# jmhb0/view_neti

Hardware: AMD Instinct MI355X
Metric: TI train steps/sec (SD-1.5 512^2 bs=4 per GPU) (higher is better)
Workload: dtype f16; 1 GPU; learnable_mode 0, sd15 shapes, 512x512 fp16, bs=4/GPU, grad_accum 1, full train step (VAE+16xCLIP+UNet fwd/bwd+AdamW); global_batch=4, parallelism=dp1, rccl_ranks=1, hipgraph=True

## Files before the change

### view_neti_amd/csrc/gemm8.hip

```cpp
#include <type_traits>

#include "common.h"
#include "gemm_args.h"

namespace {

constexpr int BM = 256, NT = 512;
constexpr int HALF_BYTES = 128 * 128;
constexpr int GN_IMG = 5;

#define VN_WAIT_VM(n) asm volatile("s_waitcnt vmcnt(" #n ")" ::: "memory")
#define VN_WAIT_LGKM0() asm volatile("s_waitcnt lgkmcnt(0)" ::: "memory")

template <int BN, int EPI, bool CONV, bool HALO = false>
__global__ __launch_bounds__(NT) void gemm8_kernel(GemmArgs g) {
  static_assert(BN == 256 || BN == 128, "tile width");
  static_assert(!HALO || (BN == 128 && CONV), "the halo-patch loop exists for the 256x128 convolution tile");
  constexpr int PATCH_STRIDE = 41 * 1024;
  constexpr bool H42 = HALO && BN == 128;
  constexpr int NJB = BN / 128;
  constexpr int HB_BYTES = (BN / 2) * 128;
  constexpr int HB_DMA = BN / 128;
  constexpr int NBUF = BN == 256 ? 2 : 3;
  constexpr int BUF_BYTES = 2 * HALF_BYTES + 2 * HB_BYTES;
// ... 633 lines not shown
        }
      }
      if (EPI == 2 && e_gate) {
        const long long go = (long long)m * g.ld_gate + (e_geglu == 2 ? 2 * n : n);
        gv[u] = as_half8(vn_buf_load16_once(rsG, ok ? (uint32_t)(go * 2) : VN_OOB));
        gv2[u] = as_half8(vn_buf_load16_once(rsG, (ok && e_geglu == 2) ? (uint32_t)(go * 2 + 16) : VN_OOB));
      }
    }
#pragma unroll
    for (int u = 0; u < U; ++u) {
      const int r = r_first + RPP * (it0 + u);
      const int m = rowmem(r);
      const bool valid = m < g.M && n < g.N;
      if (gn && !gn_one) {
        int img = gn_img;
        if (valid) {
          img = (int)((float)m * rcp_gnhw);
          const int rem = m - img * g.gn_hw;
          img += rem >= g.gn_hw ? 1 : (rem < 0 ? -1 : 0);
        }
        if (__any(img != gn_img)) {
          gn_flush();
          gn_img = img;
        }
      }
      if (!valid) continue;
      half8 v = cv[u];
      if (full_chunk) {
        if (EPI >= 1 && e_rowadd) {
          v = vn_add8(v, av[u]);
        }
        if (Rb) {
          v = vn_add8(v, rv[u]);
        }
        if (e_geglu == 2) {
#pragma unroll
          for (int c2 = 0; c2 < 2; ++c2) {
            const half8 pre = c2 == 0 ? gv[u] : gv2[u];
            half8 o;
#pragma unroll
            for (int e = 0; e < 4; ++e) {
              const float d = (float)v[4 * c2 + e], hh = (float)pre[e], gg = (float)pre[4 + e];
              float cdf, xpdf;
              vn_gelu_parts(gg, cdf, xpdf);
              o[e] = (half_t)(d * gg * cdf);
              o[4 + e] = (half_t)(d * hh * (cdf + xpdf));
            }
            vn_st16_wt(rsC, (uint32_t)(((long long)m * g.ldc + 2 * n + 8 * c2) * 2), o);
          }
          continue;
        }
        if (e_gate) {
#pragma unroll
          for (int e = 0; e < 8; ++e) v[e] = (half_t)((float)v[e] * act_grad((float)gv[u][e], g.gate_act));
        }
        if (e_geglu == 1 || (e_C2 && e_geglu == 0)) vn_st16_wt_saved(rsC, (uint32_t)(((long long)m * g.ldc + n) * 2), v);
        else vn_st16_wt(rsC, (uint32_t)(((long long)m * g.ldc + n) * 2), v);
        if (e_geglu == 1) {
          half4 o2;
#pragma unroll
          for (int e = 0; e < 4; ++e) o2[e] = (half_t)((float)v[e] * vn_gelu_erf((float)v[4 + e]));
          *reinterpret_cast<half4*>(e_C2 + (long long)m * g.ldc2 + (n >> 1)) = o2;
        }
        if (gn) {
          {
            const half2v one2 = {(half_t)1.f, (half_t)1.f};
#pragma unroll
            for (int e = 0; e < 8; e += 2) {
              const half2v p2 = {v[e], v[e + 1]};
              if (e < gn_split) {
                s_lo = VN_FDOT2(p2, one2, s_lo);
                q_lo = VN_FDOT2(p2, p2, q_lo);
              } else {
                s_hi = VN_FDOT2(p2, one2, s_hi);
                q_hi = VN_FDOT2(p2, p2, q_hi);
              }
            }
          }
        }
        if (e_C2 && e_geglu == 0) {
          half8 o2;
#pragma unroll
          for (int e = 0; e < 8; ++e) o2[e] = (half_t)apply_act((float)v[e], g.act2);
          vn_st16_wt(rsC2, (uint32_t)(((long long)m * g.ldc2 + n) * 2), o2);
        }
      } else {
        const half_t* radd = e_rowadd ? e_rowadd + (long long)(m / g.rows_per_group) * g.ld_rowadd + n : nullptr;
        for (int e = 0; e < 8 && n + e < g.N; ++e) {
          float x = (float)v[e];
          if (radd) x = (float)(half_t)(x + (float)radd[e]);
          if (Rb) x = (float)(half_t)(x + (float)Rb[(long long)m * g.ldr + n + e]);
          if (e_gate) x = (float)(half_t)(x * act_grad((float)e_gate[(long long)m * g.ld_gate + n + e], g.gate_act));
          Cb[(long long)m * g.ldc + n + e] = (half_t)x;
          if (e_C2) e_C2[(long long)m * g.ldc2 + n + e] = (half_t)apply_act((float)(half_t)x, g.act2);
          if (gn) {
            const float xs = (float)(half_t)x;
            if (e < gn_split) {
              s_lo += xs;
              q_lo += xs * xs;
            } else {
              s_hi += xs;
              q_hi += xs * xs;
            }
          }
        }
      }
    }
  }
  if (gn_one) {
    float v4[4] = {s_lo, q_lo, s_hi, q_hi};
#pragma unroll
    for (int k = 0; k < 4; ++k) {
      v4[k] += __shfl_xor(v4[k], 32);
      v4[k] += __shfl_xor(v4[k], 16);
    }
    static_assert(CPR == 16 || !HALO, "the halo tile is 128 columns wide");
    float* tab = reinterpret_cast<float*>(smem + LDS_BYTES);
    if (lane < 16) *reinterpret_cast<f32x4*>(tab + (wave * 16 + lane) * 4) = f32x4{v4[0], v4[1], v4[2], v4[3]};
    __syncthreads();
    if (tid < 32) {
      const int col = tid >> 1, half = tid & 1;
      float sv = 0.f, qv = 0.f;
#pragma unroll
      for (int w8 = 0; w8 < 8; ++w8) {
        sv += tab[(w8 * 16 + col) * 4 + 2 * half];
        qv += tab[(w8 * 16 + col) * 4 + 2 * half + 1];
      }
      const int nc = n0 + col * 8;
      const int glo = nc / g.gn_cpg;
      const int split = (glo + 1) * g.gn_cpg - nc;
      if (nc < g.N && (half == 0 || split < 8)) {
        const int slot = tile_m % g.gn_slots;
        vn_u64* dst = reinterpret_cast<vn_u64*>(e_gn_sums) + (((long long)hb * g.gn_slots + slot) * g.gn_G + glo + half) * 4;
        vn_fx_add2(dst, sv, qv);
      }
    }
  } else if (gn) {
    gn_flush();
    __syncthreads();
    const int slot = tile_m % g.gn_slots;
    for (int i = tid; i < GN_IMG * GN_NG; i += NT) {
      const vn_u64* src = gacc + 4 * i;
      if ((src[0] | src[1] | src[2] | src[3]) == 0) continue;
      const int img = gn_img0 + i / GN_NG, grp = gn_g0t + i % GN_NG;
      vn_u64* dst = reinterpret_cast<vn_u64*>(e_gn_sums) + (((long long)img * g.gn_slots + slot) * g.gn_G + grp) * 4;
#pragma unroll
      for (int w = 0; w < 4; ++w) atomicAdd(dst + w, src[w]);
    }
  }
}

inline int epilogue_level8(const GemmArgs& g) {
  if (g.gate_src || g.C2 || g.geglu || g.act) return 2;
  return (g.gn_sums || g.rowadd) ? 1 : 0;
}

}

int vneti_launch_gemm8(void* gemm_args, int bn, int halo, hipStream_t st) {
  GemmArgs& g = *reinterpret_cast<GemmArgs*>(gemm_args);
  if (g.out_f32 || (g.conv_mode && (g.ups || (g.conv_mode == 2 && g.stride == 2))) ||
      (g.M >= (1 << 24) && (g.conv_mode || g.rowadd || g.gn_sums)))
    return VNETI_EUNSUP;
  if (halo && (bn != 128 || g.conv_mode < 1 || g.conv_mode > 2 || g.stride != 1 || g.pad_t != 1 || g.pad_l != 1 || g.Hi != g.Ho ||
               g.Wi != g.Wo || (g.Ho & 15) || (g.Wo & 15) || (g.Ci & 63) || g.K != 9 * g.Ci || !g.korder ||
               g.batch != 1 || g.M != (g.M / (g.Ho * g.Wo)) * g.Ho * g.Wo))
    return VNETI_EUNSUP;
  if (halo && g.ksplit > 1) {
    const int nchunk = g.Ci / 64, cps = cdiv(nchunk, g.ksplit);
    g.kt_per_split = 9 * cps;
    g.ksplit = cdiv(nchunk, cps);
  }
  g.tiles_m = cdiv(g.M, BM);
  g.tiles_n = cdiv(g.N, bn);
  const dim3 grid(g.tiles_m * g.tiles_n, g.batch, g.ksplit), block(NT);
  const int epi = epilogue_level8(g);
#define VN_GO(E, C)                                                                        \
  do {                                                                                     \
    if (bn == 256) hipLaunchKernelGGL((gemm8_kernel<256, E, C>), grid, block, 0, st, g);   \
    else hipLaunchKernelGGL((gemm8_kernel<128, E, C>), grid, block, 0, st, g);             \
  } while (0)
#define VN_GO_HALO(E) hipLaunchKernelGGL((gemm8_kernel<128, E, true, true>), grid, block, 0, st, g)
  if (halo) {
    if (epi == 2) VN_GO_HALO(2); else if (epi == 1) VN_GO_HALO(1); else VN_GO_HALO(0);
  } else if (g.conv_mode) {
    if (epi == 2) VN_GO(2, true); else if (epi == 1) VN_GO(1, true); else VN_GO(0, true);
  } else {
    if (epi == 2) VN_GO(2, false); else if (epi == 1) VN_GO(1, false); else VN_GO(0, false);
  }
#undef VN_GO
#undef VN_GO_HALO
  return vneti_check_launch("gemm8_kernel");
}
```

### view_neti_amd/csrc/gemm_conv.hip

```cpp
#include "common.h"
#include "gemm_args.h"
#include "../../include/vneti.h"

namespace {

template <int BM, int BN, int WM, int WN, bool F32OUT, bool DMA, int NSTG = 2, int EPI = 2, bool CONV = true>
__global__ __launch_bounds__((BM / WM) * (BN / WN) * 64) void gemm_kernel(
    const half_t* pA, const half_t* pB, uint32_t p_a_bytes, uint32_t p_b_bytes, int p_lda, int p_ldb, int pM, int pN, int pK,
    int p_tiles_m, int p_tiles_n, int p_split_conv , const GemmArgs gfull) {
  GemmArgs g = gfull;
  g.A = pA;
  g.B = pB;
  g.a_bytes = p_a_bytes;
  g.b_bytes = p_b_bytes;
  g.lda = p_lda;
  g.ldb = p_ldb;
  g.M = pM;
  g.N = pN;
  g.K = pK;
  g.tiles_m = p_tiles_m;
  g.tiles_n = p_tiles_n;
  g.kt_per_split = p_split_conv & 0xffff;
  g.ksplit = (p_split_conv >> 16) & 0xff;
  g.conv_mode = p_split_conv >> 24;
// ... 466 lines not shown
              s_lo += x;
              q_lo += x * x;
            } else {
              s_hi += x;
              q_hi += x * x;
            }
          }
        }
        if (e_C2 && e_geglu == 0) {
          half8 o2;
#pragma unroll
          for (int e = 0; e < 8; ++e) o2[e] = (half_t)apply_act((float)v[e], g.act2);
          vn_st16_wt(rsC2, (uint32_t)(((long long)m * g.ldc2 + n) * 2), o2);
        }
      } else {
        for (int e = 0; e < 8 && n + e < g.N; ++e) {
          float x = (float)v[e];
          if (radd) x = (float)(half_t)(x + (float)radd[e]);
          if (Rb) x = (float)(half_t)(x + (float)Rb[(long long)m * g.ldr + n + e]);
          if (e_gate) x = (float)(half_t)(x * act_grad((float)e_gate[(long long)m * g.ld_gate + n + e], g.gate_act));
          Cb[(long long)m * g.ldc + n + e] = (half_t)x;
          if (e_C2) e_C2[(long long)m * g.ldc2 + n + e] = (half_t)apply_act((float)(half_t)x, g.act2);
          if (gn) {
            const float xs = (float)(half_t)x;
            if (e < gn_split) {
              s_lo += xs;
              q_lo += xs * xs;
            } else {
              s_hi += xs;
              q_hi += xs * xs;
            }
          }
        }
      }
    }
    if (gn) {
      gn_flush();
      __syncthreads();
      const int slot = tile_m % g.gn_slots;
      for (int i = tid; i < GN_IMG * GN_NG; i += NT) {
        const vn_u64* src = gacc + 4 * i;
        if ((src[0] | src[1] | src[2] | src[3]) == 0) continue;
        const int img = gn_img0 + i / GN_NG, grp = gn_g0t + i % GN_NG;
        vn_u64* dst = reinterpret_cast<vn_u64*>(e_gn_sums) + (((long long)img * g.gn_slots + slot) * g.gn_G + grp) * 4;
#pragma unroll
        for (int w = 0; w < 4; ++w) atomicAdd(dst + w, src[w]);
      }
    }
  }
}

__global__ __launch_bounds__(256) void splitk_reduce_kernel(
    float* p_ws, void* pC, const float* p_bias, const void* p_resid, const half_t* p_rowadd, int pM, int pN, int p_batch,
    int p_ksplit, int p_ldc, int p_ldr, const GemmArgs gfull) {
  GemmArgs g = gfull;
  g.ws = p_ws;
  g.C = pC;
  g.bias = p_bias;
  g.resid = p_resid;
  g.rowadd = p_rowadd;
  g.M = pM;
  g.N = pN;
  g.batch = p_batch;
  g.ksplit = p_ksplit;
  g.ldc = p_ldc;
  g.ldr = p_ldr;
  const unsigned n4 = (unsigned)(g.N + 3) / 4;
  const unsigned gid = blockIdx.x * 256u + threadIdx.x;
  const unsigned total = (unsigned)g.batch * (unsigned)g.M * n4;
  if (gid >= total) return;
  const unsigned row = gid / n4;
  const int c = (int)(gid - row * n4) * 4;
  const int bz = g.batch > 1 ? (int)(row / (unsigned)g.M) : 0;
  const int m = (int)(row - (unsigned)bz * (unsigned)g.M);
  const int ne = min(4, g.N - c);
  const long long zstride = (long long)g.batch * g.M * g.N;
  const float* p0 = g.ws + ((long long)bz * g.M + m) * g.N + c;
  if ((g.N & 3) == 0 && ((g.ldc | g.ldr | g.ld_rowadd | g.ld_gate | g.ldc2) & 3) == 0) {
    const long long co = (long long)bz * g.strideC + (long long)m * g.ldc + c;
    const long long ro = (long long)bz * g.strideC + (long long)m * g.ldr + c;
    f32x4 bv = {0.f, 0.f, 0.f, 0.f}, rf = {0.f, 0.f, 0.f, 0.f};
    half4 rh = {0, 0, 0, 0}, ra = {0, 0, 0, 0}, gt = {0, 0, 0, 0};
    if (g.bias) bv = *reinterpret_cast<const f32x4*>(g.bias + c);
    if (g.resid) {
      if (g.out_f32) rf = *reinterpret_cast<const f32x4*>(reinterpret_cast<const float*>(g.resid) + ro);
      else rh = *reinterpret_cast<const half4*>(reinterpret_cast<const half_t*>(g.resid) + ro);
    }
    if (g.rowadd) ra = *reinterpret_cast<const half4*>(g.rowadd + (long long)(m / g.rows_per_group) * g.ld_rowadd + c);
    if (g.gate_src) gt = *reinterpret_cast<const half4*>(g.gate_src + (long long)m * g.ld_gate + c);
    f32x4 v = {0.f, 0.f, 0.f, 0.f};
    int z = 0;
    for (; z + 4 <= g.ksplit; z += 4) {
      const f32x4 t0 = *reinterpret_cast<const f32x4*>(p0 + (z + 0) * zstride);
      const f32x4 t1 = *reinterpret_cast<const f32x4*>(p0 + (z + 1) * zstride);
      const f32x4 t2 = *reinterpret_cast<const f32x4*>(p0 + (z + 2) * zstride);
      const f32x4 t3 = *reinterpret_cast<const f32x4*>(p0 + (z + 3) * zstride);
      v += t0;
      v += t1;
      v += t2;
      v += t3;
    }
    for (; z < g.ksplit; ++z) v += *reinterpret_cast<const f32x4*>(p0 + z * zstride);
    float x[4];
#pragma unroll
    for (int e = 0; e < 4; ++e) {
      x[e] = v[e] * g.alpha;
      if (g.bias) x[e] += bv[e];
      x[e] = apply_act(x[e], g.act);
    }
    if (g.out_f32) {
      f32x4 o = {x[0], x[1], x[2], x[3]};
      if (g.resid) o += rf;
      vn_st16_wt(vn_make_rsrc(g.C, 0x7fffffffu), (uint32_t)(co * 4), o);
    } else {
      half4 o, o2;
#pragma unroll
      for (int e = 0; e < 4; ++e) {
        float y = (float)(half_t)x[e];
        if (g.rowadd) y = (float)(half_t)(y + (float)ra[e]);
        if (g.resid) y = (float)(half_t)(y + (float)rh[e]);
        if (g.gate_src) y = (float)(half_t)(y * act_grad((float)gt[e], g.gate_act));
        o[e] = (half_t)y;
        o2[e] = (half_t)apply_act((float)(half_t)y, g.act2);
      }
      *reinterpret_cast<half4*>(reinterpret_cast<half_t*>(g.C) + co) = o;
      if (g.C2) *reinterpret_cast<half4*>(g.C2 + (long long)m * g.ldc2 + c) = o2;
    }
    return;
  }
  float v[4] = {0.f, 0.f, 0.f, 0.f};
  for (int z = 0; z < g.ksplit; ++z) {
    const float* p = p0 + z * zstride;
    for (int e = 0; e < ne; ++e) v[e] += p[e];
  }
  for (int e = 0; e < ne; ++e) {
    float x = v[e] * g.alpha;
    if (g.bias) x += g.bias[c + e];
    x = apply_act(x, g.act);
    if (g.out_f32) {
      if (g.resid) x += reinterpret_cast<const float*>(g.resid)[(long long)bz * g.strideC + (long long)m * g.ldr + c + e];
      reinterpret_cast<float*>(g.C)[(long long)bz * g.strideC + (long long)m * g.ldc + c + e] = x;
    } else {
      x = (float)(half_t)x;
      if (g.rowadd) x = (float)(half_t)(x + (float)g.rowadd[(long long)(m / g.rows_per_group) * g.ld_rowadd + c + e]);
      if (g.resid)
        x = (float)(half_t)(x + (float)reinterpret_cast<const half_t*>(g.resid)[(long long)bz * g.strideC + (long long)m * g.ldr + c + e]);
      if (g.gate_src) x = (float)(half_t)(x * act_grad((float)g.gate_src[(long long)m * g.ld_gate + c + e], g.gate_act));
      reinterpret_cast<half_t*>(g.C)[(long long)bz * g.strideC + (long long)m * g.ldc + c + e] = (half_t)x;
      if (g.C2) g.C2[(long long)m * g.ldc2 + c + e] = (half_t)apply_act((float)(half_t)x, g.act2);
    }
  }
}

inline int epilogue_level(const GemmArgs& g) {
  if (g.gate_src || g.C2 || g.geglu || g.act) return 2;
  return (g.gn_sums || g.rowadd) ? 1 : 0;
}

template <int BM, int BN, int WM, int WN, bool F32OUT, bool DMA, int NSTG>
void launch_variant(const GemmArgs& g, dim3 grid, hipStream_t st) {
  const dim3 block((BM / WM) * (BN / WN) * 64);
#define VN_GO(E, C)                                                                                                        \
  hipLaunchKernelGGL((gemm_kernel<BM, BN, WM, WN, F32OUT, DMA, NSTG, E, C>), grid, block, 0, st, g.A, g.B, g.a_bytes, g.b_bytes, \
                     (int)g.lda, (int)g.ldb, g.M, g.N, g.K, g.tiles_m, g.tiles_n, g.kt_per_split | (g.ksplit << 16) | (g.conv_mode << 24), g)
  if constexpr (F32OUT) {
    if (g.conv_mode) { if (g.act) VN_GO(2, true); else VN_GO(0, true); }
    else { if (g.act) VN_GO(2, false); else VN_GO(0, false); }
  } else {
    const int epi = epilogue_level(g);
    if (g.conv_mode) { if (epi == 2) VN_GO(2, true); else if (epi == 1) VN_GO(1, true); else VN_GO(0, true); }
    else { if (epi == 2) VN_GO(2, false); else if (epi == 1) VN_GO(1, false); else VN_GO(0, false); }
  }
#undef VN_GO
}

inline void launch_reduce(const GemmArgs& g, hipStream_t st) {
  if (g.ksplit > 1) {
    long long total = (long long)g.batch * g.M * ((g.N + 3) / 4);
    hipLaunchKernelGGL(splitk_reduce_kernel, dim3((unsigned)cdivl(total, 256)), dim3(256), 0, st, g.ws, g.C, g.bias, g.resid,
                       g.rowadd, g.M, g.N, g.batch, g.ksplit, (int)g.ldc, (int)g.ldr, g);
  }
}

template <int BM, int BN, int WM, int WN, bool DMA>
int launch_cfg(GemmArgs& g, bool f32out, hipStream_t st) {
  g.tiles_m = cdiv(g.M, BM);
  g.tiles_n = cdiv(g.N, BN);
  dim3 grid(g.tiles_m * g.tiles_n, g.batch, g.ksplit);
  if (f32out) launch_variant<BM, BN, WM, WN, true, DMA, 2>(g, grid, st);
  else launch_variant<BM, BN, WM, WN, false, DMA, 2>(g, grid, st);
  launch_reduce(g, st);
  return vneti_check_launch("gemm_kernel");
}

template <int BM, int BN, int WM, int WN, int NSTG = 3>
int launch_cfg_ring(GemmArgs& g, bool f32out, hipStream_t st) {
  g.tiles_m = cdiv(g.M, BM);
  g.tiles_n = cdiv(g.N, BN);
  dim3 grid(g.tiles_m * g.tiles_n, g.batch, g.ksplit);
  if (f32out) launch_variant<BM, BN, WM, WN, true, true, NSTG>(g, grid, st);
  else launch_variant<BM, BN, WM, WN, false, true, NSTG>(g, grid, st);
  launch_reduce(g, st);
  return vneti_check_launch("gemm_kernel");
}

template <int BM, int BN, int WM, int WN, bool DMA>
int launch_cfg_f16(GemmArgs& g, hipStream_t st) {
  g.tiles_m = cdiv(g.M, BM);
  g.tiles_n = cdiv(g.N, BN);
  dim3 grid(g.tiles_m * g.tiles_n, g.batch, g.ksplit);
  launch_variant<BM, BN, WM, WN, false, DMA, 2>(g, grid, st);
  launch_reduce(g, st);
  return vneti_check_launch("gemm_kernel");
}

struct TileDims {
  int bm, bn;
};
constexpr int kMaxTile = 18;
constexpr TileDims kTiles[kMaxTile + 1] = {{0, 0},     {128, 128}, {128, 64},  {64, 64},  {256, 128}, {256, 256}, {256, 128}, {256, 128},
                                          {256, 128}, {128, 128}, {128, 128}, {128, 64},  {64, 64},   {128, 128}, {128, 64},  {64, 64},
                                          {256, 256}, {256, 128}, {256, 128}};

int select_tile(int M, int N, int batch) {
  long long t256 = (long long)cdiv(M, 256) * cdiv(N, 128) * batch;
  long long t128 = (long long)cdiv(M, 128) * cdiv(N, 128) * batch;
  long long t12864 = (long long)cdiv(M, 128) * cdiv(N, 64) * batch;
  if (N <= 64) return (M >= 2048) ? 2 : 3;
  (void)t256;
  if (t128 >= 384) return 1;
  if (t12864 >= 384) return 2;
  return 3;
}

int select_ksplit(int M, int N, int K, int batch, int tile, long long ws_floats) {
  if (ws_floats <= 0) return 1;
  const int nk = K / 64;
  long long tiles = (long long)cdiv(M, kTiles[tile].bm) * cdiv(N, kTiles[tile].bn) * batch;
  if (tiles >= 256 || nk < 16) return 1;
  int s = (int)(512 / tiles);
  if (s > nk / 8) s = nk / 8;
  if (s > 16) s = 16;
  while (s > 1 && (long long)s * batch * M * N > ws_floats) --s;
  return s < 2 ? 1 : s;
}

}

extern "C" int vneti_gemm_select_tile(int M, int N, int batch) { return select_tile(M, N, batch > 0 ? batch : 1); }

extern "C" int vneti_gemm_select_split(int M, int N, int K, int batch, int tile_hint, long long workspace_bytes) {
  if (batch <= 0) batch = 1;
  int cfg = tile_hint >= 100 ? tile_hint - 100 : tile_hint;
  if (cfg == 0) cfg = select_tile(M, N, batch);
  if (cfg < 1 || cfg > kMaxTile || K % 64 != 0) return -1;
  int ks = select_ksplit(M, N, K, batch, cfg, workspace_bytes / 4);
  const int nk = K / 64;
  if (ks > nk) ks = nk;
  if (ks < 1) ks = 1;
  return cdiv(nk, cdiv(nk, ks));
}

extern "C" int vneti_gemm_f16(const vneti_gemm_desc* d, void* stream) {
  VN_REQUIRE(d != nullptr, "gemm: null descriptor");
  VN_REQUIRE(d->A && d->B && d->C, "gemm: null operand pointer");
  VN_REQUIRE(d->M > 0 && d->N > 0 && d->K > 0, "gemm: bad shape M=%d N=%d K=%d", d->M, d->N, d->K);
  VN_REQUIRE(d->K % 64 == 0, "gemm: K=%d must be a multiple of 64", d->K);
  VN_REQUIRE(d->ldb % 8 == 0, "gemm: ldb=%lld must be a multiple of 8", d->ldb);
  int batch = d->batch > 0 ? d->batch : 1;
  GemmArgs g;
  memset(&g, 0, sizeof(g));
  g.A = (const half_t*)d->A;
  g.B = (const half_t*)d->B;
  g.C = d->C;
  g.bias = d->bias;
  g.rowadd = (const half_t*)d->rowadd;
  g.resid = d->resid;
  g.gate_src = (const half_t*)d->gate_src;
  g.ld_gate = d->ld_gate;
  g.gate_act = d->gate_act;
  g.C2 = (half_t*)d->C2;
  g.ldc2 = d->ldc2;
  g.act2 = d->act2;
  g.gn_sums = (float*)d->gn_sums;
  g.gn_hw = d->gn_hw;
  g.gn_cpg = d->gn_cpg;
  g.gn_G = d->gn_groups;
  g.gn_slots = d->gn_slots;
  g.geglu = d->geglu;
  g.lda = d->lda;
  g.ldb = d->ldb;
  g.ldc = d->ldc;
  g.ld_rowadd = d->ld_rowadd;
  g.ldr = d->ldr;
  g.strideA = d->strideA;
  g.strideB = d->strideB;
  g.strideC = d->strideC;
  g.M = d->M;
  g.N = d->N;
  g.K = d->K;
  g.batch = batch;
  g.rows_per_group = d->rows_per_group > 0 ? d->rows_per_group : 1;
  g.alpha = d->alpha;
  g.act = d->act;
  g.out_f32 = d->out_f32 ? 1 : 0;
  g.conv_mode = d->conv_mode;
  long long a_bytes;
  if (d->conv_mode == 0) {
    VN_REQUIRE(d->lda % 8 == 0, "gemm: lda=%lld must be a multiple of 8", d->lda);
    a_bytes = ((long long)(d->M - 1) * d->lda + d->K) * 2;
  } else {
    VN_REQUIRE(d->conv_mode == 1 || d->conv_mode == 2, "gemm: bad conv_mode %d", d->conv_mode);
    VN_REQUIRE(d->Ci > 0 && d->Ci % 64 == 0, "conv: Ci=%d must be a multiple of 64", d->Ci);
    VN_REQUIRE(d->K == 9 * d->Ci, "conv: K=%d must equal 9*Ci=%d", d->K, 9 * d->Ci);
    VN_REQUIRE(d->stride == 1 || d->stride == 2, "conv: stride %d unsupported", d->stride);
    VN_REQUIRE(d->Ho > 0 && d->Wo > 0 && d->M % (d->Ho * d->Wo) == 0, "conv: M=%d not a multiple of Ho*Wo", d->M);
    VN_REQUIRE(d->ldx % 8 == 0, "conv: ldx must be a multiple of 8");
    VN_REQUIRE(!(d->ups && d->conv_mode != 1), "conv: fused upsample only in forward gather mode");
    VN_REQUIRE(!(d->ups && d->stride != 1), "conv: fused upsample needs stride 1");
    g.Hi = d->Hi;
    g.Wi = d->Wi;
    g.Ci = d->Ci;
    g.Ho = d->Ho;
    g.Wo = d->Wo;
    g.stride = d->stride;
    g.pad_t = d->pad_t;
    g.pad_l = d->pad_l;
    g.ups = d->ups;
    g.ldx2 = (int)(d->ldx * 2);
    VN_REQUIRE(!d->conv_korder || d->Ci % 64 == 0, "conv: conv_korder=1 needs Ci=%d to be a multiple of 64", d->Ci);
    g.korder = d->conv_korder ? 1 : 0;
    long long nb = d->M / (d->Ho * d->Wo);
    a_bytes = nb * d->Hi * d->Wi * d->ldx * 2;
  }
  long long b_bytes = ((long long)(d->N - 1) * d->ldb + d->K) * 2;
  VN_REQUIRE(a_bytes < 0x7fffffffLL && b_bytes < 0x7fffffffLL, "gemm: operand larger than 2 GiB");
  g.a_bytes = (uint32_t)a_bytes;
  g.b_bytes = (uint32_t)b_bytes;
  if (!d->out_f32) {
    VN_REQUIRE(d->ldc % 8 == 0 || d->N < 8, "gemm: ldc=%lld must be a multiple of 8", d->ldc);
  }
  VN_REQUIRE_OUT("gemm C", vn_out_bytes(d->M, d->ldc, d->N, d->out_f32 ? 4 : 2, batch, d->strideC));
  if (d->C2) VN_REQUIRE_OUT("gemm C2", vn_out_bytes(d->M, d->ldc2, d->geglu == 1 ? d->N / 2 : d->N, 2));
  hipStream_t st = (hipStream_t)stream;
  bool f32 = d->out_f32 != 0;
  VN_REQUIRE(!(f32 && d->rowadd), "gemm: rowadd is only supported for f16 output");
  if (d->gate_src || d->C2) {
    VN_REQUIRE(!f32 && batch == 1, "gemm: gate/C2 epilogues need f16 output and batch 1");
    VN_REQUIRE(!d->gate_src || (d->gate_act >= 1 && d->gate_act <= 3 && d->ld_gate % 8 == 0), "gemm: bad gate arguments");
    VN_REQUIRE(!d->C2 || (d->act2 >= 0 && d->act2 <= 3 && d->ldc2 % 8 == 0), "gemm: bad C2 arguments");
  }

  if (d->geglu) {
    VN_REQUIRE(d->geglu == 1 || d->geglu == 2, "gemm: geglu must be 0, 1 or 2");
    VN_REQUIRE(!f32 && batch == 1 && d->N % 8 == 0, "gemm: geglu needs f16 output, batch 1 and N %% 8 == 0");
    VN_REQUIRE(d->split_k == 1, "gemm: geglu needs split_k = 1 (it lives in the fused epilogue)");
    VN_REQUIRE(!d->gn_sums, "gemm: geglu and gn_sums are exclusive");
    if (d->geglu == 1) {
      VN_REQUIRE(d->C2 && d->ldc2 % 4 == 0 && !d->gate_src, "gemm: geglu forward needs C2 ([M][N/2]) and no gate");
    } else {
      VN_REQUIRE(d->gate_src && d->ld_gate % 8 == 0 && !d->C2 && !d->resid && !d->rowadd,
                 "gemm: geglu backward needs gate_src ([M][2N] saved pre-activation) and a plain epilogue");
      VN_REQUIRE(d->ldc % 8 == 0, "gemm: geglu backward writes [M][2N]: ldc %% 8");
    }
  }
  if (d->gn_sums) {
    VN_REQUIRE(!f32 && batch == 1, "gemm: gn_sums needs f16 output and batch 1");
    VN_REQUIRE(d->gn_hw >= 64 && d->gn_cpg >= 4 && d->gn_groups > 0 && d->gn_slots > 0 && d->N == d->gn_cpg * d->gn_groups &&
                   d->M % d->gn_hw == 0 && (d->gn_cpg >= 8 || d->gn_cpg == 4),
               "gemm: bad gn_sums geometry hw=%d cpg=%d G=%d", d->gn_hw, d->gn_cpg, d->gn_groups);
    VN_REQUIRE(d->split_k == 1, "gemm: gn_sums needs split_k = 1 (the statistics live in the fused epilogue)");
  }

  int cfg = d->tile_hint;
  bool dma = true;
  if (cfg >= 100) {
    dma = false;
    cfg -= 100;
  }
  if (cfg == 0) cfg = select_tile(d->M, d->N, batch);
  VN_REQUIRE(cfg >= 1 && cfg <= kMaxTile, "gemm: unknown tile_hint %d", d->tile_hint);
  if (cfg == 18 &&
      (d->conv_mode < 1 || d->conv_mode > 2 || d->stride != 1 || d->ups || d->pad_t != 1 || d->pad_l != 1 || d->Hi != d->Ho ||
       d->Wi != d->Wo || (d->Ho & 15) || (d->Wo & 15) || (d->Ci & 63) || !d->conv_korder || batch != 1 || f32))
    cfg = 17;
  if (cfg == 18 && d->gn_sums && (d->gn_cpg & 1)) cfg = 17;
  if ((cfg == 16 || cfg == 17) && (!dma || (d->conv_mode && (d->ups || (d->conv_mode == 2 && d->stride == 2))) ||
                    (d->gn_sums && (d->gn_cpg & 1)) ||
                    (d->M >= (1 << 24) && (d->conv_mode || d->rowadd || d->gn_sums)))) cfg = cfg == 16 ? 5 : 7;
  if ((cfg == 5 || cfg == 16) && f32) cfg = 4;
  if (cfg == 17 && f32) cfg = 7;
  if ((cfg == 6 || cfg == 7) && !dma) cfg = 4;
  if (cfg >= 10 && !dma) cfg = kTiles[cfg].bm == 128 ? (kTiles[cfg].bn == 128 ? 1 : 2) : 3;
  long long ws_floats = d->workspace ? d->workspace_bytes / 4 : 0;
  int ks = d->split_k;
  if (ks == 0) ks = select_ksplit(d->M, d->N, d->K, batch, cfg, ws_floats);
  if (ks < 1) ks = 1;
  const int nk = d->K / 64;
  if (ks > nk) ks = nk;
  if (ks > 1) {
    VN_REQUIRE(d->workspace && (long long)ks * batch * d->M * d->N <= ws_floats,
               "gemm: split_k=%d needs %lld workspace bytes", ks, (long long)ks * batch * d->M * d->N * 4);
    VN_REQUIRE(batch == 1 || (d->strideC != 0), "gemm: batched split-K needs strideC");
    VN_REQUIRE((long long)batch * d->M * ((d->N + 3) / 4) < 0x7fffffffLL, "gemm: split-K output larger than 2^31 chunks");
    VN_REQUIRE_OUT("gemm split-K workspace", (long long)ks * batch * d->M * d->N * 4);
  }
  if (cfg == 18 && ks > d->Ci / 64) ks = d->Ci / 64;
  g.ksplit = ks;
  g.kt_per_split = cdiv(nk, ks);
  g.ksplit = cdiv(nk, g.kt_per_split);
  VN_REQUIRE(g.ksplit <= 255 && g.kt_per_split <= 0xffff, "gemm: split_k=%d / K=%d out of range", g.ksplit, d->K);
  g.ws = (float*)d->workspace;

#define LAUNCH(BM, BN, WM, WN) \
  return dma ? launch_cfg<BM, BN, WM, WN, true>(g, f32, st) : launch_cfg<BM, BN, WM, WN, false>(g, f32, st)
  switch (cfg) {
    case 1: LAUNCH(128, 128, 64, 64);
    case 2: LAUNCH(128, 64, 64, 32);
    case 3: LAUNCH(64, 64, 32, 32);
    case 4: LAUNCH(256, 128, 64, 64);
    case 6: return launch_cfg_ring<256, 128, 64, 64>(g, f32, st);
    case 7: return launch_cfg_ring<256, 128, 64, 32>(g, f32, st);
    case 8: LAUNCH(256, 128, 64, 32);
    case 9: LAUNCH(128, 128, 64, 32);
    case 10: return launch_cfg_ring<128, 128, 64, 32>(g, f32, st);
    case 11: return launch_cfg_ring<128, 64, 64, 32>(g, f32, st);
    case 12: return launch_cfg_ring<64, 64, 32, 32>(g, f32, st);
    case 13: return launch_cfg_ring<128, 128, 64, 32, 4>(g, f32, st);
    case 14: return launch_cfg_ring<128, 64, 64, 32, 4>(g, f32, st);
    case 15: return launch_cfg_ring<64, 64, 32, 32, 4>(g, f32, st);
    case 16:
    case 17:
    case 18: {
      const int rc = vneti_launch_gemm8(&g, cfg == 16 ? 256 : 128, cfg == 18 ? 1 : 0, st);
      if (rc != VNETI_OK) return rc;
      launch_reduce(g, st);
      return vneti_check_launch("gemm8_kernel");
    }
    default:
      return dma ? launch_cfg_f16<256, 256, 64, 64, true>(g, st) : launch_cfg_f16<256, 256, 64, 64, false>(g, st);
  }
#undef LAUNCH
}
```

### view_neti_amd/engine/schedule.py

```python
from __future__ import annotations

from functools import partial
from typing import Dict, List

import torch

from .. import lib, ops, packing


class T:

    __slots__ = ("v", "g", "gw", "rows", "cols", "children", "need_grad", "producer")

    def __init__(self, v, g=None, need_grad=True):
        self.v = v
        self.g = g
        self.gw = False
        self.rows, self.cols = v.shape
        self.children: List["T"] = []
        self.need_grad = need_grad
        self.producer = None


def rup(x, m):
# ... 113 lines not shown
        if cache_path and os.path.exists(cache_path) and not cache:
            import ast
            import json
            for k, v in json.load(open(cache_path)).items():
                cache[ast.literal_eval(k)] = tuple(v)
        n_before = len(cache)
        from .. import parallel
        share = parallel.sharing_picks() and parallel._dist() is not None
        rank0 = (not share) or parallel._dist().get_rank() == 0
        if share and not rank0:
            cache.update(parallel.share_from_rank0(None))
        for lst in (self.fwd_pre, self.fwd, self.bwd):
            for idx, f in enumerate(lst):
                if getattr(f, "func", None) is not ops.gemm or f.keywords.get("tile_hint"):
                    continue
                key = self._gemm_key(f)
                conv = f.keywords.get("conv")
                try_cm = bool(conv) and not conv.get("ups") and not conv.get("korder") and \
                    not (conv["mode"] == 2 and conv["stride"] == 2) and conv["Ci"] % 64 == 0 and conv["Ci"] >= 128
                B_cm = None
                if key not in cache:
                    best, best_t = (0, 0, 0), float("inf")
                    M_, N_, K_ = key[:3]
                    halo_ok = try_cm and conv["mode"] in (1, 2) and conv["stride"] == 1 and conv["pad_t"] == 1 and conv["pad_l"] == 1 \
                        and conv["Ho"] % 16 == 0 and conv["Wo"] % 16 == 0 and conv["Hi"] == conv["Ho"] and conv["Wi"] == conv["Wo"]
                    variants = [(h, 0) for h in candidates if h != 18] + \
                        ([(h, 1) for h in candidates if h in (16, 17) or (h == 18 and halo_ok)] if try_cm else [])
                    if try_cm:
                        B_cm = packing._chunk_major(f.args[1], f.args[1].shape[0], conv["Ci"])
                    for h, ko in variants:
                        bm, bn = self._TILE_DIMS[h % 100]
                        tiles = -(-M_ // bm) * -(-N_ // bn) * key[3]
                        sks = (0, 1) + (tuple(x for x in (2, 3, 4, 6, 8, 12)
                                              if x * 8 <= K_ // 64 and tiles * x <= 1024 and x * key[3] * M_ * N_ <= 16 * 2 ** 20)
                                        if tiles < 256 else ())
                        if f.keywords.get("geglu"):
                            sks = (1,)
                        for sk in sks:
                            kw = dict(f.keywords)
                            kw["tile_hint"], kw["split_k"] = h, sk
                            args = f.args
                            if ko:
                                kw["conv"] = dict(conv, korder=1)
                                args = (f.args[0], B_cm) + tuple(f.args[2:])
                            ops.gemm(*args, **kw)
                            ops.gemm(*args, **kw)
                            if cold is None:
                                s, e = torch.cuda.Event(enable_timing=True), torch.cuda.Event(enable_timing=True)
                                s.record()
                                for _ in range(reps):
                                    ops.gemm(*args, **kw)
                                e.record()
                                e.synchronize()
                                t = s.elapsed_time(e)
                            else:
                                ts = []
                                for _ in range(cold_reps):
                                    cold.fill_(0)
                                    if warm_a:
                                        args[0].add_(0)
                                    s, e = torch.cuda.Event(enable_timing=True), torch.cuda.Event(enable_timing=True)
                                    s.record()
                                    ops.gemm(*args, **kw)
                                    e.record()
                                    e.synchronize()
                                    ts.append(s.elapsed_time(e))
                                t = sorted(ts)[len(ts) // 2]
                            if t < best_t:
                                best, best_t = (h, sk, ko), t
                    cache[key] = best
                pick = tuple(cache[key]) + (0,) * (3 - len(cache[key]))
                kw = dict(f.keywords)
                kw["tile_hint"], kw["split_k"] = pick[0], pick[1]
                if pick[2] and try_cm:
                    if B_cm is None:
                        B_cm = packing._chunk_major(f.args[1], f.args[1].shape[0], conv["Ci"])
                    kw["conv"] = dict(conv, korder=1)
                    self.bytes += B_cm.numel() * B_cm.element_size()
                    f_cm = partial(ops.gemm, f.args[0], B_cm, *f.args[2:], **f.keywords)
                    if getattr(f, "side", False):
                        f_cm.side = True
                    f = f_cm
                lst[idx] = self._rebound(f, ops.gemm, kw)
        if share and rank0:
            parallel.share_from_rank0(dict(cache))
        if cache_path and len(cache) != n_before and parallel.world_info()[0] == 0:
            import json
            tmp = f"{cache_path}.{os.getpid()}.tmp"
            with open(tmp, "w") as fh:
                json.dump({repr(k): list(v) for k, v in cache.items()}, fh)
            os.replace(tmp, cache_path)

    def bind_workspace(self):
        for lst in (self.fwd_pre, self.fwd, self.bwd):
            for idx, f in enumerate(lst):
                fn = getattr(f, "func", None)
                if fn is ops.gemm or fn is ops.attn_bwd_dkv:
                    kw = dict(f.keywords)
                    kw["workspace"] = self.ws_side if getattr(f, "side", False) else self.ws
                    lst[idx] = self._rebound(f, fn, kw)

    @staticmethod
    def _rebound(f, fn, kw):
        p = partial(fn, *f.args, **kw)
        if getattr(f, "side", False):
            p.side = True
        return p

    def _side(self, launch):
        launch.side = True
        if self.ws_side is None:
            self.ws_side = self._buf((4 * 2 ** 20,), torch.float32)
        return launch

    GN_SLOTS = 8

    def _produced(self, t: T):
        t.producer = len(self.fwd) - 1
        return t

    GN2_MAX = 512

    def _gn2_slice(self):
        if not hasattr(self, "_gn2_arena"):
            self._gn2_arena = self._buf((self.GN2_MAX, self.B, self.GN_SLOTS, self.groups, 4), torch.int64, zero=True)
            self._gn2_used = 0
        assert self._gn2_used < self.GN2_MAX
        self._gn2_used += 1
        return self._gn2_arena[self._gn2_used - 1]

    def fuse_gn_stats(self, fuse: bool = True):
        n = self._fuse_gn_stats() if fuse else 0
        if getattr(self, "_gn2_used", 0):
            self.fwd.insert(0, self._gn2_arena[:self._gn2_used].zero_)
        return n

    def _fuse_gn_stats(self):
        import os
        if os.environ.get("VNETI_NO_GN_FUSE"):
            return 0
        S, G, B = self.GN_SLOTS, self.groups, self.B
        todo = []
        for rec in self._gn_fusable:
            f = self.fwd[rec["prod"]]
            kw = f.keywords
            hw, Cc = rec["hw"], rec["C"]
            cpg = Cc // G
            if getattr(f, "func", None) is ops.conv3x3_in:
                if hw % 256 == 0 and cpg % 4 == 0 and 128 % cpg == 0 and kw.get("gn_sums") is None:
                    todo.append(rec)
                continue
            if getattr(f, "func", None) is not ops.gemm or kw.get("batch"):
                continue
            if kw.get("split_k") != 1:
                M_, N_, K_ = self._gemm_key(f)[:3]
                ws = kw.get("workspace")
                wsb = ws.numel() * ws.element_size() if ws is not None else 0
                if ops.gemm_select_split(M_, N_, K_, 1, kw.get("tile_hint") or 0, wsb) != 1:
                    continue
            if hw < 64 or not (cpg >= 8 or cpg == 4) or kw.get("gn_sums") is not None:
                continue
            todo.append(rec)
        if not todo:
            return 0
        self.gn_sums = self._buf((len(todo), B, S, G, 4), torch.int64, zero=True)
        for i, rec in enumerate(todo):
            sums = self.gn_sums[i]
            f = self.fwd[rec["prod"]]
            kw = dict(f.keywords)
            kw.update(gn_sums=sums, gn_hw=rec["hw"], gn_groups=G, gn_slots=S)
            if f.func is ops.gemm:
                kw.update(split_k=1)
            self.fwd[rec["prod"]] = self._rebound(f, f.func, kw)
            g = rec["gn"]
            self.fwd[rec["idx"]] = partial(ops.groupnorm_fwd_sums, rec["x"], rec["y"], g["gamma"], g["beta"], sums, S,
                                           g["mean"], g["rstd"], B, rec["hw"], rec["C"], G, rec["eps"], rec["silu"])
        arena = self.gn_sums
        self.fwd.insert(0, arena.zero_)
        self._gn_fusable = []
        return len(todo)

    def _gn(self, x: T, name, w, eps, silu):
        Cc = x.cols
        hw = x.rows // self.B
        rec = dict(kind="gn", x=x, gamma=self._w32(w[name + ".weight"]), beta=self._w32(w[name + ".bias"]),
                   mean=self._buf((self.B * self.groups,), torch.float32),
                   rstd=self._buf((self.B * self.groups,), torch.float32), silu=silu, hw=hw)
        y = self._buf((x.rows, Cc))
        import os
        if os.environ.get("VNETI_GN_3L"):
            self.fwd.append(partial(ops.groupnorm_fwd, x.v, y, rec["gamma"], rec["beta"], rec["mean"], rec["rstd"],
                                    self.gn_ws, self.B, hw, Cc, self.groups, eps, silu))
        else:
            self.fwd.append(partial(ops.groupnorm_fwd_2l, x.v, y, rec["gamma"], rec["beta"], self._gn2_slice(),
                                    self.GN_SLOTS, rec["mean"], rec["rstd"], self.B, hw, Cc, self.groups, eps, silu))
            if self.need_backward:
                rec["bsums"] = self._gn2_slice()
        if x.producer is not None:
            self._gn_fusable.append(dict(idx=len(self.fwd) - 1, prod=x.producer, gn=rec, x=x.v, y=y, hw=hw, C=Cc,
                                         eps=eps, silu=silu))
        return y, rec

    def _gn_bwd_fn(self, rec, dy):
        x = rec["x"]
        if "bsums" not in rec:
            fn = lambda out, accum: ops.groupnorm_bwd(dy, x.v, rec["gamma"], rec["beta"], rec["mean"], rec["rstd"], out,
                                                      self.gn_ws, self.B, rec["hw"], x.cols, self.groups,
                                                      rec["silu"], accum=accum)
        else:
            fn = lambda out, accum: ops.groupnorm_bwd_2l(dy, x.v, rec["gamma"], rec["beta"], rec["mean"], rec["rstd"], out,
                                                         rec["bsums"], self.GN_SLOTS, self.gn_ws, self.B, rec["hw"], x.cols,
                                                         self.groups, rec["silu"], accum=accum)
        fn.vn_cost = ("GroupNorm(+SiLU) bwd", 5.0 * self.B * rec["hw"] * x.cols * 2)
        return fn

    def _conv_desc(self, Hi, Wi, Ci, Ho, Wo, stride, pad, ups, ldx, mode=1):
        return dict(mode=mode, Hi=Hi, Wi=Wi, Ci=Ci, Ho=Ho, Wo=Wo, stride=stride, pad_t=pad, pad_l=pad, ups=ups,
                    ldx=ldx, korder=1 if (packing.KORDER_CM and Ci % 64 == 0) else 0)

    def _resnet(self, x: T, cin, cout, name, w, out_view, h, wd, need_dx=True):
        M = x.rows
        n1, gn1 = self._gn(x, name + "norm1", w, self.eps, True)
        w1 = self._w16(packing.conv3x3_fwd(w[name + "conv1.weight"]))
        b1 = self._w32(w[name + "conv1.bias"])
        radd = None
        if name in self.temb_off:
            off, n = self.temb_off[name]
            radd = self.temb_all[:, off:off + n]
        h1 = T(self._buf((M, cout)))
        self.fwd.append(partial(ops.gemm, n1, w1, h1.v, bias=b1, rowadd=radd, rows_per_group=h * wd, M=M,
                                conv=self._conv_desc(h, wd, cin, h, wd, 1, 1, 0, cin)))
        self._produced(h1)
        n2, gn2 = self._gn(h1, name + "norm2", w, self.eps, True)
        w2 = self._w16(packing.conv3x3_fwd(w[name + "conv2.weight"]))
        b2 = self._w32(w[name + "conv2.bias"])
        out = T(out_view if out_view is not None else self._buf((M, cout)))
        wsc = None
        if cin != cout:
            wsc = self._w16(w[name + "conv_shortcut.weight"].reshape(cout, cin))
            bsc = self._w32(w[name + "conv_shortcut.bias"])
            sc_buf = self._buf((M, cout))
            self.fwd.append(partial(ops.gemm, x.v, wsc, sc_buf, bias=bsc))
            resid = sc_buf
        else:
            resid = x.v
        self.fwd.append(partial(ops.gemm, n2, w2, out.v, bias=b2, resid=resid, M=M,
                                conv=self._conv_desc(h, wd, cout, h, wd, 1, 1, 0, cout)))
        self._produced(out)
        rec = dict(kind="resnet", x=x, out=out, h1=h1, gn1=gn1, gn2=gn2, cin=cin, cout=cout, h=h, wd=wd,
                   need_dx=need_dx, name=name)
        if self.need_backward and need_dx:
            rec["w2d"] = self._w16(packing.conv3x3_dgrad(w[name + "conv2.weight"]))
            rec["w1d"] = self._w16(packing.conv3x3_dgrad(w[name + "conv1.weight"]))
            if wsc is not None:
                rec["wscd"] = self._w16(w[name + "conv_shortcut.weight"].reshape(cout, cin).t())
        self.tape.append(rec)
        return out

    def _resnet_bwd(self, r):
        if not r["need_dx"]:
            return
        x, out, h, wd, cin, cout = r["x"], r["out"], r["h"], r["wd"], r["cin"], r["cout"]
        M = x.rows
        dout = out.g
        assert out.gw, f"resnet {r['name']}: output gradient was never produced"
        dn2 = self._tmp("dA", M, cout)
        self.bwd.append(partial(ops.gemm, dout, r["w2d"], dn2, M=M,
                                conv=self._conv_desc(h, wd, cout, h, wd, 1, 1, 0, dout.stride(0), mode=2)))
        dh1 = self._tmp("dB", M, cout)
        self.bwd.append(partial(self._gn_bwd_fn(r["gn2"], dn2), dh1, None))
        dn1 = self._tmp("dC", M, cin)
        self.bwd.append(partial(ops.gemm, dh1, r["w1d"], dn1, M=M,
                                conv=self._conv_desc(h, wd, cout, h, wd, 1, 1, 0, cout, mode=2)))
        if "wscd" in r:
            self._contrib_gemm(x, dout, r["wscd"])
            self._contrib(x, self._gn_bwd_fn(r["gn1"], dn1))
        else:
            self._contrib(x, self._gn_bwd_fn(r["gn1"], dn1), extra=dout)

    def _ln(self, xv, name, w):
        rows, Cc = xv.shape
        rec = dict(x=xv, gamma=self._w32(w[name + ".weight"]), beta=self._w32(w[name + ".bias"]),
                   mean=self._buf((rows,), torch.float32), rstd=self._buf((rows,), torch.float32))
        y = self._buf((rows, Cc))
        self.fwd.append(partial(ops.layernorm_fwd, xv, y, rec["gamma"], rec["beta"], rec["mean"], rec["rstd"], 1e-5))
        return y, rec

    def _ln_bwd(self, rec, dy, dx, accum, f16_copy=None):
        ops.layernorm_bwd(dy, rec["x"], rec["gamma"], rec["mean"], rec["rstd"], dx, accum=accum, f16_copy=f16_copy)

    def _downsample(self, x: T, Cc, name, w, out_view, h, wd, pad=1):
        M = x.rows // 4
        wf = self._w16(packing.conv3x3_fwd(w[name + "weight"]))
        b = self._w32(w[name + "bias"])
        out = T(out_view if out_view is not None else self._buf((M, Cc)))
        self.fwd.append(partial(ops.gemm, x.v, wf, out.v, bias=b, M=M,
                                conv=self._conv_desc(h, wd, Cc, h // 2, wd // 2, 2, pad, 0, x.v.stride(0))))
        self._produced(out)
        rec = dict(kind="down", x=x, out=out, C=Cc, h=h, wd=wd, pad=pad)
        if self.need_backward:
            rec["wd_"] = self._w16(packing.conv3x3_dgrad(w[name + "weight"]))
        self.tape.append(rec)
        return out

    def _downsample_bwd(self, r):
        x, out, Cc, h, wd = r["x"], r["out"], r["C"], r["h"], r["wd"]
        assert out.gw
        desc = self._conv_desc(h // 2, wd // 2, Cc, h, wd, 2, r["pad"], 0, out.g.stride(0), mode=2)
        self._contrib_gemm(x, out.g, r["wd_"], M=x.rows, conv=desc)

    def forward_pre(self):
        for f in self.fwd_pre:
            f()

    def forward_main(self):
        for f in self.fwd:
            f()

    def forward(self):
        self.forward_pre()
        self.forward_main()

    def _run(self, lst):
        side = None
        main = None
# ... 17 lines not shown
```

Before: 39.20 steps/s.

## Fuse GroupNorm statistics into the split-K reduce kernel so split-K GEMMs stay split

Adds a split-K reduce kernel that applies the full epilogue and also accumulates per-image, per-group GroupNorm sums into the fixed-point atomic arena. The GEMM epilogue now skips GN statistics when split-K is active. The scheduler no longer forces split_k=1 or excludes split-K GEMMs from GN-stat fusion; it filters only on leading dimensions being multiples of 4. This lets GEMMs that benefit from split-K keep their parallelism while still avoiding a separate GN statistics pass. The cost is extra shared-memory atomics and global atomics in the reduce step.

```diff
diff --git a/view_neti_amd/csrc/gemm8.hip b/view_neti_amd/csrc/gemm8.hip
--- a/view_neti_amd/csrc/gemm8.hip
+++ b/view_neti_amd/csrc/gemm8.hip
@@ -809,7 +809,7 @@
 
 inline int epilogue_level8(const GemmArgs& g) {
   if (g.gate_src || g.C2 || g.geglu || g.act) return 2;
-  return (g.gn_sums || g.rowadd) ? 1 : 0;
+  return ((g.gn_sums && g.ksplit == 1) || g.rowadd) ? 1 : 0;
 }
 
 }
diff --git a/view_neti_amd/csrc/gemm_conv.hip b/view_neti_amd/csrc/gemm_conv.hip
--- a/view_neti_amd/csrc/gemm_conv.hip
+++ b/view_neti_amd/csrc/gemm_conv.hip
@@ -642,9 +642,100 @@
   }
 }
 
+constexpr int RGN_NG = 64 / 4 + 2;
+__global__ __launch_bounds__(256) void splitk_reduce_gn_kernel(const GemmArgs g) {
+  __shared__ vn_u64 gacc[2 * RGN_NG * 4];
+  const int tid = threadIdx.x;
+  for (int i = tid; i < 2 * RGN_NG * 4; i += 256) gacc[i] = 0;
+  __syncthreads();
+  const int n4 = g.N >> 2;
+  const int cx = blockIdx.x * 16 + (tid & 15);
+  const int c = cx * 4;
+  const bool cvalid = cx < n4;
+  const int rb = blockIdx.y * 16;
+  const int img0 = rb / g.gn_hw;
+  const int g0 = (blockIdx.x * 64) / g.gn_cpg;
+  const int glo = c / g.gn_cpg;
+  const int split = (glo + 1) * g.gn_cpg - c;
+  const long long zstride = (long long)g.M * g.N;
+  f32x4 bv = {0.f, 0.f, 0.f, 0.f};
+  if (cvalid && g.bias) bv = *reinterpret_cast<const f32x4*>(g.bias + c);
+  float s0 = 0.f, q0 = 0.f, s1 = 0.f, q1 = 0.f;
+  float t0 = 0.f, r0 = 0.f, t1 = 0.f, r1 = 0.f;
+  const int m = rb + (tid >> 4);
+  if (cvalid && m < g.M) {
+    const long long co = (long long)m * g.ldc + c;
+    half4 rh = {0, 0, 0, 0}, ra = {0, 0, 0, 0}, gt = {0, 0, 0, 0};
+    if (g.resid) rh = *reinterpret_cast<const half4*>(reinterpret_cast<const half_t*>(g.resid) + (long long)m * g.ldr + c);
+    if (g.rowadd) ra = *reinterpret_cast<const half4*>(g.rowadd + (long long)(m / g.rows_per_group) * g.ld_rowadd + c);
+    if (g.gate_src) gt = *reinterpret_cast<const half4*>(g.gate_src + (long long)m * g.ld_gate + c);
+    const float* p0 = g.ws + (long long)m * g.N + c;
+    f32x4 v = {0.f, 0.f, 0.f, 0.f};
+    int z = 0;
+    for (; z + 4 <= g.ksplit; z += 4) {
+      const f32x4 a0 = *reinterpret_cast<const f32x4*>(p0 + (z + 0) * zstride);
+      const f32x4 a1 = *reinterpret_cast<const f32x4*>(p0 + (z + 1) * zstride);
+      const f32x4 a2 = *reinterpret_cast<const f32x4*>(p0 + (z + 2) * zstride);
+      const f32x4 a3 = *reinterpret_cast<const f32x4*>(p0 + (z + 3) * zstride);
+      v += a0;
+      v += a1;
+      v += a2;
+      v += a3;
+    }
+    for (; z < g.ksplit; ++z) v += *reinterpret_cast<const f32x4*>(p0 + z * zstride);
+    half4 o, o2;
+    float sl = 0.f, ql = 0.f, sh = 0.f, qh = 0.f;
+#pragma unroll
+    for (int e = 0; e < 4; ++e) {
+      float x = v[e] * g.alpha;
+      if (g.bias) x += bv[e];
+      x = apply_act(x, g.act);
+      float y = (float)(half_t)x;
+      if (g.rowadd) y = (float)(half_t)(y + (float)ra[e]);
+      if (g.resid) y = (float)(half_t)(y + (float)rh[e]);
+      if (g.gate_src) y = (float)(half_t)(y * act_grad((float)gt[e], g.gate_act));
+      o[e] = (half_t)y;
+      o2[e] = (half_t)apply_act((float)(half_t)y, g.act2);
+      const float xs = (float)o[e];
+      if (e < split) {
+        sl += xs;
+        ql += xs * xs;
+      } else {
+        sh += xs;
+        qh += xs * xs;
+      }
+    }
+    *reinterpret_cast<half4*>(reinterpret_cast<half_t*>(g.C) + co) = o;
+    if (g.C2) *reinterpret_cast<half4*>(g.C2 + (long long)m * g.ldc2 + c) = o2;
+    if (m / g.gn_hw == img0) {
+      s0 += sl, q0 += ql, s1 += sh, q1 += qh;
+    } else {
+      t0 += sl, r0 += ql, t1 += sh, r1 += qh;
+    }
+  }
+  if (cvalid) {
+    vn_u64* a = gacc + (glo - g0) * 4;
+    if (s0 != 0.f || q0 != 0.f) vn_fx_add2(a, s0, q0);
+    if (s1 != 0.f || q1 != 0.f) vn_fx_add2(a + 4, s1, q1);
+    a += RGN_NG * 4;
+    if (t0 != 0.f || r0 != 0.f) vn_fx_add2(a, t0, r0);
+    if (t1 != 0.f || r1 != 0.f) vn_fx_add2(a + 4, t1, r1);
+  }
+  __syncthreads();
+  const int slot = blockIdx.y % g.gn_slots;
+  for (int i = tid; i < 2 * RGN_NG; i += 256) {
+    const vn_u64* src = gacc + 4 * i;
+    if ((src[0] | src[1] | src[2] | src[3]) == 0) continue;
+    const int img = img0 + i / RGN_NG, grp = g0 + i % RGN_NG;
+    vn_u64* dst = reinterpret_cast<vn_u64*>(g.gn_sums) + (((long long)img * g.gn_slots + slot) * g.gn_G + grp) * 4;
+#pragma unroll
+    for (int w = 0; w < 4; ++w) atomicAdd(dst + w, src[w]);
+  }
+}
+
 inline int epilogue_level(const GemmArgs& g) {
   if (g.gate_src || g.C2 || g.geglu || g.act) return 2;
-  return (g.gn_sums || g.rowadd) ? 1 : 0;
+  return ((g.gn_sums && g.ksplit == 1) || g.rowadd) ? 1 : 0;
 }
 
 template <int BM, int BN, int WM, int WN, bool F32OUT, bool DMA, int NSTG>
@@ -665,7 +756,9 @@
 }
 
 inline void launch_reduce(const GemmArgs& g, hipStream_t st) {
-  if (g.ksplit > 1) {
+  if (g.ksplit > 1 && g.gn_sums) {
+    hipLaunchKernelGGL(splitk_reduce_gn_kernel, dim3((unsigned)cdiv(g.N / 4, 16), (unsigned)cdiv(g.M, 16)), dim3(256), 0, st, g);
+  } else if (g.ksplit > 1) {
     long long total = (long long)g.batch * g.M * ((g.N + 3) / 4);
     hipLaunchKernelGGL(splitk_reduce_kernel, dim3((unsigned)cdivl(total, 256)), dim3(256), 0, st, g.ws, g.C, g.bias, g.resid,
                        g.rowadd, g.M, g.N, g.batch, g.ksplit, (int)g.ldc, (int)g.ldr, g);
@@ -859,7 +952,6 @@
     VN_REQUIRE(d->gn_hw >= 64 && d->gn_cpg >= 4 && d->gn_groups > 0 && d->gn_slots > 0 && d->N == d->gn_cpg * d->gn_groups &&
                    d->M % d->gn_hw == 0 && (d->gn_cpg >= 8 || d->gn_cpg == 4),
                "gemm: bad gn_sums geometry hw=%d cpg=%d G=%d", d->gn_hw, d->gn_cpg, d->gn_groups);
-    VN_REQUIRE(d->split_k == 1, "gemm: gn_sums needs split_k = 1 (the statistics live in the fused epilogue)");
   }
 
   int cfg = d->tile_hint;
@@ -901,6 +993,11 @@
   g.ksplit = cdiv(nk, g.kt_per_split);
   VN_REQUIRE(g.ksplit <= 255 && g.kt_per_split <= 0xffff, "gemm: split_k=%d / K=%d out of range", g.ksplit, d->K);
   g.ws = (float*)d->workspace;
+  if (d->gn_sums && g.ksplit > 1) {
+    VN_REQUIRE(d->N % 4 == 0 && ((d->ldc | d->ldr | d->ld_rowadd | d->ld_gate | d->ldc2) & 3) == 0,
+               "gemm: gn_sums under split-K needs N and every leading dimension a multiple of 4");
+    VN_REQUIRE(d->M <= 16 * 65535, "gemm: gn_sums under split-K: M=%d too large for the reduce grid", d->M);
+  }
 
 #define LAUNCH(BM, BN, WM, WN) \
   return dma ? launch_cfg<BM, BN, WM, WN, true>(g, f32, st) : launch_cfg<BM, BN, WM, WN, false>(g, f32, st)
diff --git a/view_neti_amd/engine/schedule.py b/view_neti_amd/engine/schedule.py
--- a/view_neti_amd/engine/schedule.py
+++ b/view_neti_amd/engine/schedule.py
@@ -289,12 +289,10 @@
                 continue
             if getattr(f, "func", None) is not ops.gemm or kw.get("batch"):
                 continue
-            if kw.get("split_k") != 1:
-                M_, N_, K_ = self._gemm_key(f)[:3]
-                ws = kw.get("workspace")
-                wsb = ws.numel() * ws.element_size() if ws is not None else 0
-                if ops.gemm_select_split(M_, N_, K_, 1, kw.get("tile_hint") or 0, wsb) != 1:
-                    continue
+            lds = [kw.get("ldc") or f.args[2].stride(0), Cc] + \
+                [kw[k].stride(0) for k in ("resid", "rowadd", "gate", "out2") if kw.get(k) is not None]
+            if any(v % 4 for v in lds):
+                continue
             if hw < 64 or not (cpg >= 8 or cpg == 4) or kw.get("gn_sums") is not None:
                 continue
             todo.append(rec)
@@ -306,8 +304,6 @@
             f = self.fwd[rec["prod"]]
             kw = dict(f.keywords)
             kw.update(gn_sums=sums, gn_hw=rec["hw"], gn_groups=G, gn_slots=S)
-            if f.func is ops.gemm:
-                kw.update(split_k=1)
             self.fwd[rec["prod"]] = self._rebound(f, f.func, kw)
             g = rec["gn"]
             self.fwd[rec["idx"]] = partial(ops.groupnorm_fwd_sums, rec["x"], rec["y"], g["gamma"], g["beta"], sums, S,
```

After: 39.20 steps/s (median of 4 runs). No clear change (+0.0%).
